# ChristophReich1996/Multi-StyleGAN

Measured on AMD Instinct MI355X. Metric: training images/sec (G+D step, 256^2, seq=3x2ch), higher is better.
Workload: dtype bf16

## Files before the change

include/msg_hip.h:

```cpp
#ifndef MSG_HIP_H
#define MSG_HIP_H

#ifdef __cplusplus
extern "C" {
#endif

enum { MSG_OK = 0, MSG_EINVAL = -1, MSG_EUNSUPPORTED = -2, MSG_ELAUNCH = -3 };
enum { MSG_F32 = 0, MSG_BF16 = 1, MSG_F16 = 2, MSG_F64 = 3, MSG_F32_SPLIT = 4 };

#define MSG_ABI_VERSION 5
int msg_abi_version(void);
const char* msg_build_arch(void);
const char* msg_strerror(int code);

int msg_upfirdn2d(const void* x, const float* fir, void* y, int dtype,
                  int major, int in_h, int in_w, int minor, int kh, int kw,
                  int up_x, int up_y, int down_x, int down_y,
                  int pad_x0, int pad_x1, int pad_y0, int pad_y1, void* stream);

int msg_upfirdn2d_pitched(const void* x, const float* fir, void* y, int dtype,
                          int major, int in_h, int in_w, int minor, int in_pitch, int kh, int kw,
                          int up_x, int up_y, int down_x, int down_y,
                          int pad_x0, int pad_x1, int pad_y0, int pad_y1, void* stream);

// ... 119 lines not shown

long long msg_minibatch_stddev_workspace(int C, int H, int W, int groups, int dtype);
int msg_minibatch_stddev(const void* x, void* y, float* stat, float* workspace, int dtype,
                         int B, int C, int H, int W, int ldx, int ldy, int groups, float alpha, void* stream);
int msg_minibatch_stddev_backward(const void* x, const void* gy, const float* gstat, void* gx, int dtype,
                                  int B, int C, int H, int W, int ldx, int ldgy, int ldgx, int groups,
                                  float alpha, void* stream);

int msg_conv2d_fprop_act(const void* x, const void* w, void* y, int dtype,
                         int B, int IH, int IW, int Cx, int Ck, int OH, int OW, int N, int ldy,
                         int kh, int kw, int stride, int pad, long long w_batch_stride,
                         const float* act_bias, const float* noise, const float* noise_weight,
                         int noise_batch, float alpha, float scale, void* stream);
int msg_conv2d_fprop_act_mask(const void* x, const void* w, void* y, int dtype,
                              int B, int IH, int IW, int Cx, int Ck, int OH, int OW, int N, int ldy,
                              int kh, int kw, int stride, int pad, long long w_batch_stride,
                              const float* act_bias, const float* noise, const float* noise_weight,
                              int noise_batch, float alpha, float scale, unsigned char* mask, void* stream);

int msg_conv2d_fprop_residual(const void* x, const void* w, void* y, int dtype,
                              int B, int IH, int IW, int Cx, int Ck, int OH, int OW, int N, int ldy,
                              int kh, int kw, int stride, int pad, long long w_batch_stride,
                              const void* residual, int res_ld, float gain, void* stream);

long long msg_conv2d_fprop_act_backward_workspace(int dtype, int B, int IH, int IW, int Cx, int Ck, int OH, int OW,
                                                  int N, int kh, int kw, long long w_batch_stride, int has_noise);
int msg_conv2d_fprop_act_backward(const void* x, const void* w, void* y, int dtype,
                                  int B, int IH, int IW, int Cx, int Ck, int OH, int OW, int N, int ldy,
                                  int kh, int kw, int stride, int pad, long long w_batch_stride,
                                  const void* residual, int res_ld,
                                  const unsigned char* sign_mask, int mask_tile_m, int mask_tile_n,
                                  const void* sign_map, int sign_ld, float alpha, float scale,
                                  float* grad_bias, const float* noise, int noise_batch, float* grad_noise_weight,
                                  float* ws, long long ws_floats, void* stream);

int msg_act_pointwise_head(const void* x, const float* bias, const float* w, float* y, int dtype,
                           long long npix, int C, float wscale, float alpha, float scale, void* stream);
long long msg_act_pointwise_head_backward_workspace(long long npix, int C);
int msg_act_pointwise_head_backward(const void* x, const float* bias, const float* w, const float* gy, void* gx,
                                    float* grad_bias_and_w, int dtype, long long npix, int C, float wscale,
                                    float alpha, float scale, float* ws, long long ws_floats, void* stream);

int msg_linear_fprop(const float* x, const float* w, const float* bias, float* y, int M, int N, int K,
                     float gain, float bias_gain, void* stream);
int msg_linear_dgrad(const float* gy, const float* w, float* gx, int M, int N, int K, float gain, void* stream);
int msg_linear_wgrad(const float* gy, const float* x, float* gw, float* gb, int M, int N, int K,
// ... 66 lines not shown
```

multi_stylegan_amd/conv_ops.py:

```python
import math
import os
from typing import Optional, Tuple

import torch
from torch.autograd import Function

from . import _lib
from ._autograd import _derive


def _vec(dtype) -> int:
    return 8 if dtype == torch.bfloat16 else 4


def _round_up(n: int, m: int) -> int:
    return (n + m - 1) // m * m


def _padded_nhwc(b, c, h, w, dtype, device):
    cx = _round_up(c, _vec(dtype))
    buf = torch.empty((b, h, w, cx), dtype=dtype, device=device)
    if cx != c:
        buf[..., c:].zero_()
    return buf.permute(0, 3, 1, 2)[:, :c]
# ... 315 lines not shown
        return self

    def __exit__(self, *exc):
        global FP32_CONTRACTION
        FP32_CONTRACTION = self.prev
        return False

    @staticmethod
    def set(mode: str) -> None:
        fp32_contraction(mode).__enter__()


def _contraction_code(t: torch.Tensor, mode: Optional[str] = None) -> int:
    code = _lib.dtype_code(t)
    mode = FP32_CONTRACTION if mode is None else mode
    return _SPLIT_CODES[mode] if (code == _lib.MSG_F32 and mode != "exact") else code


_PLANS = {_lib.MSG_PLAN_REG: ("conv_fprop_reg", None), _lib.MSG_PLAN_DMA: ("conv_fprop_dma", None),
          _lib.MSG_PLAN_PP: ("conv_fprop_pp", None), _lib.MSG_PLAN_ROW3: ("conv_fprop_row3", 256),
          _lib.MSG_PLAN_ROW3N: ("conv_fprop_row3n", 128), _lib.MSG_PLAN_THIN: ("conv_fprop_thin", None)}
_PLAN_CACHE: dict = {}
_WGRAD_WS_CACHE: dict = {}


def _launch_fprop(x, wk, ck, bias, n, out_hw, kh, kw, stride, pad, in_up, pixel_shuffle, per_sample, c_real,
                  flops=None, act=None, residual=None, out=None, mode=None):
    dev = _lib.require_gpu(x, wk, bias)
    xv, cx = _nhwc_view(x)
    b, _, ih, iw = xv.shape
    oh, ow = out_hw
    if out is not None:
        y, ldy = _nhwc_view(out)
        if y is not out or pixel_shuffle or out.shape != (b, n, oh, ow) or out.dtype != x.dtype or n % _vec(x.dtype):
            raise _lib.MsgHipError(f"conv fprop: destination {tuple(out.shape)} / {out.stride()} for a {(b, n, oh, ow)} result")
    elif pixel_shuffle:
        y, ldy = _alloc_out(b, n // 4, 2 * oh, 2 * ow, x.dtype, dev)
    else:
        y, ldy = _alloc_out(b, n, oh, ow, x.dtype, dev)
    rows_needed = n * (1 if pixel_shuffle else kh * kw) * ck
    if per_sample:
        ws_ = wk.stride() if wk.ndim == 4 else None
        if ws_ is None or wk.shape[0] != b or ws_[0] < rows_needed or ws_[3] != 1 or \
                (wk.shape[2] > 1 and ws_[2] != wk.shape[3]) or (wk.shape[1] > 1 and ws_[1] != wk.shape[2] * wk.shape[3]):
            raise _lib.MsgHipError(f"conv fprop: per-sample weight image {tuple(wk.shape)} for batch {b}, {n} x {kh * kw} x {ck}")
    elif wk.numel() < rows_needed or not wk.is_contiguous():
        raise _lib.MsgHipError(f"conv fprop: weight image {tuple(wk.shape)} smaller than {n} x {kh * kw} x {ck}")
    wstride = wk.stride(0) if per_sample else 0
    if flops is None:
        flops = 2.0 * b * oh * ow * n * kh * kw * c_real / (in_up * in_up)
    key = "conv_fprop"
    if _lib.kernel_clock.enabled:
        plan = _lib.lib().msg_conv2d_fprop_plan(_lib.dtype_code(x), b, ih, iw, cx, ck, oh, ow, n, kh, kw, wstride)
        key = _PLANS[_lib.MSG_PLAN_REG if plan == _lib.MSG_PLAN_THIN and act is not None else plan][0]
        if x.dtype == torch.bfloat16 and bias is None and act is None and residual is None and \
                _lib.lib().msg_conv2d_fprop_upconv_eligible(b, ih, iw, cx, ck, oh, ow, n, kh, kw, stride, pad, in_up,
                                                           int(pixel_shuffle), wstride):
            key = "conv_fprop_upconv"
        if _CLOCK_SHAPES:
            key += f"|B{b} {ih}x{iw}->{oh}x{ow} {c_real}->{n} {kh}x{kw} s{stride} up{in_up}" \
                   f"{' ps' if pixel_shuffle else ''}{' per-sample' if per_sample else ''}|"
    with _lib.on_device(dev), _lib.kernel_clock.span((key, 'bf16' if x.dtype == torch.bfloat16 else 'f32'), flops):
        if residual is not None:
            assert bias is None and act is None and in_up == 1 and not pixel_shuffle
            rv, res_ld = _nhwc_view(residual[0])
            assert rv.shape == (b, n, oh, ow) and rv.dtype == x.dtype
            code = _lib.lib().msg_conv2d_fprop_residual(
                xv.data_ptr(), wk.data_ptr(), y.data_ptr(), _contraction_code(x, mode), b, ih, iw, cx, ck, oh, ow, n, ldy, kh, kw,
                stride, pad, wstride, rv.data_ptr(), res_ld, float(residual[1]), _lib.stream_of(dev))
        elif act is None:
            code = _lib.lib().msg_conv2d_fprop(
                xv.data_ptr(), wk.data_ptr(), _lib.ptr(bias), y.data_ptr(), _contraction_code(x, mode), b, ih, iw, cx, ck, oh,
                ow, n, ldy, kh, kw, stride, pad, in_up, int(pixel_shuffle), wstride, _lib.stream_of(dev))
        else:
            assert bias is None and in_up == 1 and not pixel_shuffle
            act_bias, noise, noise_w, alpha, scale = act[:5]
            _lib.require_gpu(x, act_bias, noise, noise_w)
            mask = None
            if len(act) > 5 and act[5] is not None and kh == 3 and stride == 1 and pad == 1:
                pkey = (x.dtype, b, ih, iw, cx, ck, oh, ow, n, kh, kw, wstride)
                mplan = _PLAN_CACHE.get(pkey)
                if mplan is None:
                    mplan = _PLAN_CACHE[pkey] = _lib.lib().msg_conv2d_fprop_plan(_lib.dtype_code(x), b, ih, iw, cx, ck, oh, ow,
                                                                                n, kh, kw, wstride)
                tile = _PLANS[mplan][1]
                if tile:
                    from .op_static.fused_act import sign_mask_for
                    mask = sign_mask_for(b, n, oh, ow, x.dtype, dev)
                    if mask is not None:
                        act[5].append((mask, tile, tile))
            code = _lib.lib().msg_conv2d_fprop_act_mask(
                xv.data_ptr(), wk.data_ptr(), y.data_ptr(), _contraction_code(x, mode), b, ih, iw, cx, ck, oh, ow, n, ldy, kh, kw,
                stride, pad, wstride, _lib.ptr(act_bias), _lib.ptr(noise), _lib.ptr(noise_w),
                1 if noise is None else noise.shape[0], float(alpha), float(scale), _lib.ptr(mask), _lib.stream_of(dev))
    _lib.check(code, "msg_conv2d_fprop")
    return y


def _grad_dest(param):
    if param is None or "_msg_grad_slot" not in getattr(param, "__dict__", ()):
        return None
    from .dist import grad_destination
    return grad_destination(param)


def wgrad_k_chunks(b, o, i, taps, oh, ow, per_sample, kp):
    tiles = ((o + 127) // 128) * ((i + 127) // 128) * taps * b
    if per_sample:
        return max(1, min((oh * ow) // (16 * kp), 1024 // tiles)) if tiles < 256 else 1
    k_chunks = max(1, min((oh * ow + 4 * kp - 1) // (4 * kp), (1024 + tiles - 1) // tiles))
    while b * k_chunks > 65535:
        k_chunks -= 1
    return k_chunks


def _launch_wgrad(gy, x, o, i, kh, kw, stride, pad, pixel_shuffle, per_sample, low_hw, raw=False, gain=1.0, out=None,
                  mode=None):
# ... 1293 lines not shown
```

multi_stylegan_amd/csrc/conv_dispatch.h:

```cpp
#pragma once
#include "msg_common.h"

struct ConvProblem {
    int dtype;
    int split;
    int B, IH, IW, Cx, Ck, OH, OW, N, ldy;
    int kh, kw, stride, pad, in_up, pixel_shuffle;
    long long w_batch_stride;

    bool per_sample() const { return w_batch_stride != 0; }
    int samples() const { return per_sample() ? B : 1; }
    long long mtot() const { return per_sample() ? (long long)OH * OW : (long long)B * OH * OW; }
    int esz() const { return dtype == MSG_BF16 ? 2 : 4; }
    long long x_bstride() const { return (long long)IH * IW * Cx; }
    long long y_bstride() const { return (pixel_shuffle ? 4ll : 1ll) * OH * OW * ldy; }
    long long x_bytes() const { return (long long)(per_sample() ? 1 : B) * IH * IW * Cx * esz(); }
    long long w_bytes() const { return (long long)N * kh * kw * Ck * esz(); }
    bool fits31() const { return x_bytes() < 0x7ffffff0ll && w_bytes() < 0x7ffffff0ll; }
};

enum ConvKernel {
    CONV_THIN_N, CONV_THIN_K,
    CONV_UPCONV,
    CONV_ROW3, CONV_ROW3N,
    CONV_PP,
    CONV_DMA, CONV_REG, CONV_REG_LEAN, CONV_REG_SPLIT
};

struct ConvPlan {
    ConvKernel kernel;
    int tile_m, tile_n;
    bool supported;
};

inline int conv_act_mode(const ActEpilogue* act) { return act ? act->enabled : 0; }

template <typename P>
inline void conv_fill_common(P& p, const ConvProblem& q, const ActEpilogue* act) {
    p.B = q.B; p.IH = q.IH; p.IW = q.IW; p.Cx = q.Cx; p.Ck = q.Ck; p.OH = q.OH; p.OW = q.OW; p.N = q.N; p.ldy = q.ldy;
    p.per_sample = q.per_sample();
    if (act) p.act = *act;
    p.x_bstride = q.x_bstride();
    p.w_bstride = q.w_batch_stride;
    p.y_bstride = q.y_bstride();
    p.Mtot = (int)q.mtot();
}
template <typename P>
inline void conv_fill_taps(P& p, const ConvProblem& q) {
    p.kh = q.kh; p.kw = q.kw; p.stride = q.stride; p.pad = q.pad; p.in_up = q.in_up; p.pixel_shuffle = q.pixel_shuffle;
}

ConvPlan conv_fprop_select(const ConvProblem& q, const ActEpilogue* act, bool has_bias);

bool conv_thin_eligible(const ConvProblem& q, const ActEpilogue* act, ConvPlan* plan);
void conv_thin_launch(const ConvProblem& q, const ConvPlan& plan, const void* x, const void* w, const float* bias, void* y,
                      const ActEpilogue* act, void* stream);
bool conv_upconv_eligible(const ConvProblem& q, const ActEpilogue* act, bool has_bias, ConvPlan* plan);
void conv_upconv_launch(const ConvProblem& q, const ConvPlan& plan, const void* x, const void* w, void* y, void* stream);
bool conv_row3_eligible(const ConvProblem& q, const ActEpilogue* act, bool has_bias, ConvPlan* plan);
void conv_row3_launch(const ConvProblem& q, const ConvPlan& plan, const void* x, const void* w, const float* bias, void* y,
                      const ActEpilogue* act, void* stream);
bool conv_pp_eligible(const ConvProblem& q, ConvPlan* plan);
void conv_pp_launch(const ConvProblem& q, const ConvPlan& plan, const void* x, const void* w, const float* bias, void* y,
                    const ActEpilogue* act, void* stream);

struct WgradProblem {
    int dtype, split;
    int B, IH, IW, Cx, I, OH, OW, ldgy, O, ldgw;
    int kh, kw, stride, pad, pixel_shuffle;
    int per_sample, k_chunks, oi_major;
    float gain;
    int esz() const { return dtype == MSG_BF16 ? 2 : 4; }
    long long gy_bytes() const { return (long long)(pixel_shuffle ? 4 : 1) * OH * OW * ldgy * esz(); }
    long long x_bytes() const { return (long long)IH * IW * Cx * esz(); }
    long long slab() const { return (long long)O * kh * kw * ldgw; }
// ... 36 lines not shown
```

multi_stylegan_amd/csrc/conv_fprop.hip:

```cpp
#include "conv_dispatch.h"
#include <stdlib.h>

typedef __bf16 bf16v8 __attribute__((ext_vector_type(8)));
typedef const __attribute__((address_space(1))) char* gptr_t;
typedef const __attribute__((address_space(1))) u32x4* gvec_t;
typedef __attribute__((address_space(3))) char* lds_t;

struct ConvParams {
    int B, IH, IW, Cx, Ck, OH, OW, N, ldy;
    int kh, kw, stride, pad, in_up, pixel_shuffle, per_sample;
    long long x_bstride, w_bstride, y_bstride;
    int Mtot, n_chunks, n_iters, m_tiles, n_tiles;
    ActEpilogue act;
};

constexpr int BM = 128, BN = 128, ROWB = 128;
constexpr int STAGE_BYTES = (BM + BN) * ROWB;
__device__ __attribute__((aligned(256))) unsigned int g_zero_page[16384];

__device__ __forceinline__ int swz(int row, int slot) { return row * ROWB + ((slot ^ ((row >> 1) & 7)) << 4); }

template <int SPLIT>
__device__ __forceinline__ void split_park(const u32x4& raw, char* dst) {
    uint2 pl[3];
#pragma unroll
    for (int h = 0; h < 2; ++h) {
        const float x0 = __uint_as_float(raw[2 * h]), x1 = __uint_as_float(raw[2 * h + 1]);
        const unsigned hp = (unsigned)f2bf(x0) | ((unsigned)f2bf(x1) << 16);
        const float r0 = x0 - __uint_as_float(hp << 16), r1 = x1 - __uint_as_float(hp & 0xffff0000u);
        const unsigned mp = (unsigned)f2bf(r0) | ((unsigned)f2bf(r1) << 16);
        (h ? pl[0].y : pl[0].x) = hp;
        (h ? pl[1].y : pl[1].x) = mp;
        if constexpr (SPLIT == 3) {
            const float q0 = r0 - __uint_as_float(mp << 16), q1 = r1 - __uint_as_float(mp & 0xffff0000u);
            (h ? pl[2].y : pl[2].x) = (unsigned)f2bf(q0) | ((unsigned)f2bf(q1) << 16);
        }
    }
#pragma unroll
    for (int p = 0; p < SPLIT; ++p) *reinterpret_cast<uint2*>(dst + p * 64) = pl[p];
}

template <typename T, bool DMA, int LEAN = 0, int SPLIT = 0>
__global__ __launch_bounds__(256, LEAN ? LEAN : 2) void conv_fprop_kernel(const T* __restrict__ x, const T* __restrict__ w,
                                                            T* __restrict__ y, const float* __restrict__ bias,
                                                            ConvParams p) {
    constexpr int VEC = 16 / sizeof(T);
    constexpr int BKE = ROWB / sizeof(T);
    static_assert(!LEAN || (!DMA && sizeof(T) == 2), "lean variant: bf16, register staging");
    static_assert(SPLIT == 0 || sizeof(T) == 4, "split-bf16 products are a mode of the fp32-storage kernel");
    static_assert(SPLIT == 0 || !DMA, "the split planes are written from the staging registers");
    constexpr int SROW = SPLIT ? SPLIT * 64 + 16 : ROWB;
    constexpr int STAGE = SPLIT ? (BM + BN) * SROW : STAGE_BYTES;
    constexpr bool ONE_STAGE = LEAN != 0 || SPLIT == 3;
    constexpr int SMEM_BYTES = ONE_STAGE ? (STAGE > 65536 || sizeof(T) == 2 ? STAGE : 65536) : 2 * STAGE;
    __shared__ __attribute__((aligned(16))) char smem[SMEM_BYTES];

    const int tid = threadIdx.x, lane = tid & 63, wid = tid >> 6;
    const int wm = wid >> 1, wn = wid & 1;
    const int lr = lane & 31, lh = lane >> 5;
    const unsigned L = xcd_remap(blockIdx.x, gridDim.x);
    const int n0 = (int)(L % p.n_tiles) * BN;
    const int m0 = (int)(L / p.n_tiles) * BM;
    const int bz = blockIdx.z;

    const int wid_u = __builtin_amdgcn_readfirstlane(wid);
    const int slot_phys = tid & 7;
    int row_of[4];
#pragma unroll
    for (int j = 0; j < 4; ++j) row_of[j] = DMA ? (wid * 32 + 8 * j + (lane >> 3)) : ((tid >> 3) + 32 * j);
    const int slot = DMA ? 0 : slot_phys;
    int a_ih0[4], a_iw0[4];
    long long a_boff[4];
    int a_slot[4];
// ... 40 lines not shown
#pragma unroll
        for (int j = 0; j < 4; ++j) {
            const int n = n0 + row_of[j];
            vb[j] = n < p.N ? (int)(((long long)n * taps * p.Ck + a_slot[j] * VEC) * (long long)sizeof(T)) : MSG_DMA_OOB;
        }
    }
    const bool ragged = (p.Cx % BKE) != 0;
    int ld_tap = -1, ld_chunk = p.n_chunks - 1;
    int kh_ = 0, kw_ = -1;
    int st_off[4];
#pragma unroll
    for (int j = 0; j < 4; ++j) st_off[j] = swz(row_of[j], a_slot[j]);

    f32x16 acc[2][2];
#pragma unroll
    for (int i = 0; i < 2; ++i)
#pragma unroll
        for (int j = 0; j < 2; ++j)
#pragma unroll
            for (int e = 0; e < 16; ++e) acc[i][j][e] = 0.f;

    u32x4 ra[4], rb[4];
    int dma_stage = 0;
    auto load_next = [&]() __attribute__((always_inline)) {
        if (++ld_chunk == p.n_chunks) {
            ld_chunk = 0;
            ++ld_tap;
            if (++kw_ == p.kw) { kw_ = 0; ++kh_; }
            if (p.in_up == 1) {
                const long long tap_off = ((long long)kh_ * p.IW + kw_) * p.Cx * (long long)sizeof(T);
#pragma unroll
                for (int j = 0; j < 4; ++j) {
                    const bool ok = a_ok[j] & ((unsigned)(a_ih0[j] + kh_) < (unsigned)p.IH) &
                                    ((unsigned)(a_iw0[j] + kw_) < (unsigned)p.IW);
                    pa[j] = (ok ? xbase : zbase) + (ok ? a_boff[j] + tap_off : zoff);
                    if constexpr (DMA) va[j] = ok ? (int)(a_boff[j] + tap_off) : MSG_DMA_OOB;
                }
            } else {
#pragma unroll
                for (int j = 0; j < 4; ++j) {
                    const int ih = a_ih0[j] + kh_, iw = a_iw0[j] + kw_;
                    bool ok = a_ok[j] & (ih >= 0) & (iw >= 0) & (ih % p.in_up == 0) & (iw % p.in_up == 0);
                    const int ihs = ih / p.in_up, iws = iw / p.in_up;
                    ok = ok & (ihs < p.IH) & (iws < p.IW);
                    const long long off = a_boff[j] + ((long long)(ihs - a_ih0[j]) * p.IW + (iws - a_iw0[j])) * p.Cx * (long long)sizeof(T);
                    pa[j] = (ok ? xbase : zbase) + (ok ? off : zoff);
                    if constexpr (DMA) va[j] = ok ? (int)off : MSG_DMA_OOB;
                }
            }
        }
#pragma unroll
        for (int j = 0; j < 4; ++j) {
            const bool c_bad = ragged && (ld_chunk * BKE + a_slot[j] * VEC + VEC > p.Cx);
            gptr_t a_addr = pa[j];
            if (c_bad) a_addr = zbase + zoff;
            if constexpr (DMA) {
                const unsigned la = lds0 + dma_stage * STAGE + (wid_u * 32 + 8 * j) * ROWB;
                msg_dma16(d_x, la, c_bad ? MSG_DMA_OOB : va[j], ld_chunk * ROWB);
                msg_dma16(d_w, la + BM * ROWB, vb[j], (ld_tap * p.n_chunks + ld_chunk) * ROWB);
            } else {
                ra[j] = *(gvec_t)a_addr;
                rb[j] = *(gvec_t)pb[j];
            }
            pa[j] += ROWB;
            pb[j] += ROWB;
        }
    };
    auto park = [&](int stage) __attribute__((always_inline)) {
        char* sa = smem + stage * STAGE;
        if constexpr (SPLIT != 0) {
            char* sb = sa + BM * SROW;
#pragma unroll
// ... 62 lines not shown
                            for (int pa = 0; pa <= order; ++pa)
                                acc[i][j] = __builtin_amdgcn_mfma_f32_32x32x16_bf16(bf[order - pa][j], af[pa][i], acc[i][j], 0, 0, 0);
                    }
            }
        } else {
#pragma unroll
            for (int q = 0; q < 4; ++q) {
                f32x4 fa[2], fb[2];
#pragma unroll
                for (int t = 0; t < 2; ++t) {
                    fa[t] = *reinterpret_cast<const f32x4*>(sa + swz(wm * 64 + t * 32 + lr, 4 * lh + q));
                    fb[t] = *reinterpret_cast<const f32x4*>(sb + swz(wn * 64 + t * 32 + lr, 4 * lh + q));
                }
#pragma unroll
                for (int e = 0; e < 4; ++e)
#pragma unroll
                    for (int i = 0; i < 2; ++i)
#pragma unroll
                        for (int j = 0; j < 2; ++j)
                            acc[i][j] = __builtin_amdgcn_mfma_f32_32x32x2f32(fb[j][e], fa[i][e], acc[i][j], 0, 0, 0);
            }
        }
    };
    if constexpr (ONE_STAGE) {
        load_next();
        for (int it = 0; it < p.n_iters; ++it) {
            if (it) __syncthreads();
            park(0);
            if (it + 1 < p.n_iters) load_next();
            __syncthreads();
            mma_step(smem);
        }
    } else {
        if constexpr (DMA) {
            dma_stage = 0;
            load_next();
        } else {
            load_next();
            park(0);
            if (p.n_iters > 1) load_next();
        }
        for (int it = 0; it < p.n_iters; ++it) {
            if constexpr (DMA) asm volatile("s_waitcnt vmcnt(0)" ::: "memory");
            __syncthreads();
            if constexpr (DMA) {
                if (it + 1 < p.n_iters) { dma_stage = (it + 1) & 1; load_next(); }
            } else {
                if (it + 1 < p.n_iters) park((it + 1) & 1);
                if (it + 2 < p.n_iters) load_next();
            }
            mma_step(smem + (it & 1) * STAGE);
        }
    }
    if constexpr (DMA) asm volatile("s_waitcnt vmcnt(0)" ::: "memory");
    __syncthreads();

    constexpr int PITCH = 64 * sizeof(T);
    constexpr int UNITB = 4 * sizeof(T);
    char* ep = smem + wid * (64 * PITCH);
#pragma unroll
    for (int j = 0; j < 2; ++j)
#pragma unroll
        for (int g = 0; g < 4; ++g) {
            const int unit = 8 * j + 2 * g + lh;
            float bv[4] = {0.f, 0.f, 0.f, 0.f};
            if (bias) {
                const int nb = n0 + wn * 64 + 4 * unit;
#pragma unroll
                for (int e = 0; e < 4; ++e) bv[e] = nb + e < p.N ? bias[nb + e] : 0.f;
            }
#pragma unroll
            for (int i = 0; i < 2; ++i) {
                const int row = i * 32 + lr;
                char* dstl = ep + row * PITCH + ((unit ^ (row & 15)) * UNITB);
                if constexpr (sizeof(T) == 2) {
// ... 67 lines not shown
#pragma unroll
        for (int pass = 0; pass < NPASS; ++pass)
            r[pass] = *reinterpret_cast<const u32x4*>(rbase + (long long)max(gp[pass], 0) * p.act.res_ld);
#pragma unroll
        for (int pass = 0; pass < NPASS; ++pass) v[pass] = residual_epilogue_apply<T>(v[pass], r[pass], p.act.res_gain);
    }
    T* ybase = y + (p.pixel_shuffle ? nn : n);
    if (n_ok && lim >= VEC) {
#pragma unroll
        for (int pass = 0; pass < NPASS; ++pass)
            if (gp[pass] >= 0) *reinterpret_cast<u32x4*>(ybase + (long long)gp[pass] * p.ldy) = v[pass];
    } else if (n_ok) {
#pragma unroll
        for (int pass = 0; pass < NPASS; ++pass) {
            if (gp[pass] < 0) continue;
            T tmp[VEC];
            *reinterpret_cast<u32x4*>(tmp) = v[pass];
            T* dst = ybase + (long long)gp[pass] * p.ldy;
            for (int e = 0; e < lim; ++e) dst[e] = tmp[e];
        }
    }
}

static ConvPlan conv_generic_select(const ConvProblem& q) {
    const int n_iters = q.kh * q.kw * (q.Ck / (ROWB / q.esz()));
    static const int variant = msg_tunable("MSG_CONV_VARIANT", 0);
    const bool dma = q.fits31() && (variant == 1 || (variant == 0 && n_iters >= 8));
    static const int lean_max = msg_tunable("MSG_CONV_LEAN", 4);
    ConvPlan plan{CONV_REG, BM, BN, true};
    if (q.split) plan.kernel = CONV_REG_SPLIT;
    else if (dma) plan.kernel = CONV_DMA;
    else if (q.dtype == MSG_BF16 && n_iters <= lean_max) plan.kernel = CONV_REG_LEAN;
    const long long mtot = q.mtot(), blocks = ((mtot + BM - 1) / BM) * ((q.N + BN - 1) / BN);
    plan.supported = mtot < (1ll << 31) && blocks < (1ll << 31) &&
                     (long long)(n_iters + 1) * ROWB + 128 <= 65536;
    return plan;
}

static void conv_generic_launch(const ConvProblem& q, const ConvPlan& plan, const void* x, const void* w, const float* bias, void* y,
                                const ActEpilogue* act, void* stream) {
    ConvParams p{};
    conv_fill_common(p, q, act);
    conv_fill_taps(p, q);
    p.n_chunks = q.Ck / (ROWB / q.esz());
    p.n_iters = q.kh * q.kw * p.n_chunks;
    p.m_tiles = (int)((q.mtot() + BM - 1) / BM);
    p.n_tiles = (q.N + BN - 1) / BN;
    dim3 grid((unsigned)((long long)p.m_tiles * p.n_tiles), 1, q.samples());
#define GENERIC(T, ...) hipLaunchKernelGGL((conv_fprop_kernel<T, __VA_ARGS__>), grid, dim3(256), 0, (hipStream_t)stream, \
                                           (const T*)x, (const T*)w, (T*)y, bias, p)
    const bool bf16 = q.dtype == MSG_BF16;
    if (bf16 && plan.kernel == CONV_REG_LEAN) GENERIC(bf16_t, false, 3);
    else if (bf16 && plan.kernel == CONV_DMA) GENERIC(bf16_t, true);
    else if (bf16) GENERIC(bf16_t, false);
    else if (plan.kernel == CONV_REG_SPLIT) GENERIC(float, false, 0, 3);
    else if (plan.kernel == CONV_DMA) GENERIC(float, true);
    else GENERIC(float, false);
#undef GENERIC
}

ConvPlan conv_fprop_select(const ConvProblem& q, const ActEpilogue* act, bool has_bias) {
    ConvPlan plan;
    if (conv_thin_eligible(q, act, &plan)) return plan;
    if (conv_upconv_eligible(q, act, has_bias, &plan)) return plan;
    if (conv_row3_eligible(q, act, has_bias, &plan)) return plan;
    if (conv_pp_eligible(q, &plan)) return plan;
    return conv_generic_select(q);
}

static ConvProblem conv_problem(int dtype, int B, int IH, int IW, int Cx, int Ck, int OH, int OW, int N, int ldy,
                                int kh, int kw, int stride, int pad, int in_up, int pixel_shuffle, long long w_batch_stride) {
    const int split = dtype == MSG_F32_SPLIT ? 3 : 0;
    return ConvProblem{split ? (int)MSG_F32 : dtype, split, B, IH, IW, Cx, Ck, OH, OW, N, ldy, kh, kw, stride, pad, in_up, pixel_shuffle,
                       w_batch_stride};
}
static ConvProblem conv_query_problem(int dtype, int B, int IH, int IW, int Cx, int Ck, int OH, int OW, int N, int kh, int kw,
                                      long long w_batch_stride) {
    return conv_problem(dtype, B, IH, IW, Cx, Ck, OH, OW, N, N <= 8 ? 8 : (N + 7) / 8 * 8, kh, kw, 1, kh / 2, 1, 0, w_batch_stride);
}

extern "C" int msg_conv2d_fprop_plan(int dtype, int B, int IH, int IW, int Cx, int Ck, int OH, int OW, int N,
                                     int kh, int kw, long long w_batch_stride) {
    switch (conv_fprop_select(conv_query_problem(dtype, B, IH, IW, Cx, Ck, OH, OW, N, kh, kw, w_batch_stride), nullptr, false).kernel) {
        case CONV_THIN_N: case CONV_THIN_K: return MSG_PLAN_THIN;
        case CONV_ROW3: return MSG_PLAN_ROW3;
        case CONV_ROW3N: return MSG_PLAN_ROW3N;
        case CONV_PP: return MSG_PLAN_PP;
        case CONV_UPCONV: return MSG_PLAN_PP;
        case CONV_DMA: return MSG_PLAN_DMA;
        default: return MSG_PLAN_REG;
    }
}

static int conv2d_fprop_impl(const void* x, const void* w, const float* bias, void* y, const ConvProblem& q,
                             const ActEpilogue& act, void* stream, const ConvPlan* selected = nullptr);

extern "C" int msg_conv2d_fprop(const void* x, const void* w, const float* bias, void* y, int dtype,
                                int B, int IH, int IW, int Cx, int Ck, int OH, int OW, int N, int ldy,
                                int kh, int kw, int stride, int pad, int in_up, int pixel_shuffle,
                                long long w_batch_stride, void* stream) {
    ActEpilogue act{};
    return conv2d_fprop_impl(x, w, bias, y, conv_problem(dtype, B, IH, IW, Cx, Ck, OH, OW, N, ldy, kh, kw, stride, pad, in_up,
                                                         pixel_shuffle, w_batch_stride), act, stream);
}

static bool is_row3(const ConvPlan& plan) { return plan.kernel == CONV_ROW3 || plan.kernel == CONV_ROW3N; }

extern "C" int msg_conv2d_fprop_act_mask(const void* x, const void* w, void* y, int dtype,
                                         int B, int IH, int IW, int Cx, int Ck, int OH, int OW, int N, int ldy,
                                         int kh, int kw, int stride, int pad, long long w_batch_stride,
                                         const float* act_bias, const float* noise, const float* noise_weight,
                                         int noise_batch, float alpha, float scale, unsigned char* mask, void* stream) {
    if (noise && (!noise_weight || (noise_batch != 1 && noise_batch != B))) return MSG_EINVAL;
    const ConvProblem q = conv_problem(dtype, B, IH, IW, Cx, Ck, OH, OW, N, ldy, kh, kw, stride, pad, 1, 0, w_batch_stride);
    ActEpilogue act{act_bias, noise, noise_weight, noise_batch, 1, alpha, scale, nullptr, 0, 0.f, mask};
    if (!mask) return conv2d_fprop_impl(x, w, nullptr, y, q, act, stream);
    const ConvPlan plan = conv_fprop_select(q, &act, false);
    return is_row3(plan) ? conv2d_fprop_impl(x, w, nullptr, y, q, act, stream, &plan) : (int)MSG_EUNSUPPORTED;
}

extern "C" int msg_conv2d_fprop_act(const void* x, const void* w, void* y, int dtype,
                                    int B, int IH, int IW, int Cx, int Ck, int OH, int OW, int N, int ldy,
                                    int kh, int kw, int stride, int pad, long long w_batch_stride,
                                    const float* act_bias, const float* noise, const float* noise_weight,
                                    int noise_batch, float alpha, float scale, void* stream) {
    return msg_conv2d_fprop_act_mask(x, w, y, dtype, B, IH, IW, Cx, Ck, OH, OW, N, ldy, kh, kw, stride, pad, w_batch_stride,
// ... 49 lines not shown
    act_backward_partials(q, plan, &rows, &entries);
    if (!rows) return MSG_EUNSUPPORTED;
    if (sign_mask && (mask_tile_m <= 0 || mask_tile_n <= 0 || mask_tile_n % 128 || N % mask_tile_n || (((uintptr_t)sign_mask) & 15u) ||
                      (mask_tile_m != 1 && mask_tile_m % 64) || ((long long)B * OH * OW) % mask_tile_m))
        return MSG_EINVAL;
    if (sign_map && (sign_ld < N || sign_ld % 8 || (((uintptr_t)sign_map) & 15u))) return MSG_EINVAL;
    if (residual && (res_ld < N || res_ld % 8 || (((uintptr_t)residual) & 15u))) return MSG_EINVAL;
    const bool has_noise = noise && grad_noise_weight;
    if (has_noise && noise_batch != 1 && noise_batch != B) return MSG_EINVAL;
    const long long need_b = grad_bias ? rows * N : 0, need_n = has_noise ? entries : 0;
    if (need_b + need_n > 0 && (!ws || ws_floats < need_b + need_n)) return MSG_EINVAL;
    act.residual = residual; act.res_ld = res_ld; act.res_gain = 1.f;
    act.mask = const_cast<unsigned char*>(sign_mask); act.mask_tile_m = mask_tile_m; act.mask_tile_n = mask_tile_n;
    act.sign_src = sign_map; act.sign_ld = sign_ld;
    act.noise = has_noise ? noise : nullptr; act.noise_batch = noise_batch;
    act.part_b = grad_bias ? ws : nullptr;
    act.part_n = has_noise ? ws + need_b : nullptr;
    conv_row3_launch(q, plan, x, w, nullptr, y, &act, stream);
    if (MSG_CHECK_LAUNCH() != MSG_OK) return MSG_ELAUNCH;
    return msg_bias_act_reduce_launch(act.part_b, grad_bias, N, rows, act.part_n, grad_noise_weight, entries, stream);
}

static int conv2d_fprop_impl(const void* x, const void* w, const float* bias, void* y, const ConvProblem& q,
                             const ActEpilogue& act, void* stream, const ConvPlan* selected) {
    if (q.B == 0) return MSG_OK;
    if (!x || !w || !y || q.B < 0 || q.IH <= 0 || q.IW <= 0 || q.OH <= 0 || q.OW <= 0 || q.N <= 0 || q.kh <= 0 || q.kw <= 0 ||
        q.stride <= 0 || q.in_up <= 0 || q.Cx <= 0 || q.Ck <= 0 || q.ldy <= 0)
        return MSG_EINVAL;
    if (q.dtype != MSG_F32 && q.dtype != MSG_BF16) return MSG_EUNSUPPORTED;
    const int vec = 16 / q.esz(), bke = ROWB / q.esz();
    if (q.Ck % bke || q.Cx % vec || (((uintptr_t)x | (uintptr_t)w | (uintptr_t)y) & 15u)) return MSG_EUNSUPPORTED;
    if (q.ldy % vec || (q.pixel_shuffle && (q.N % 4 || (q.N / 4) % vec))) return MSG_EUNSUPPORTED;
    if (q.in_up > 1 && q.stride != 1) return MSG_EUNSUPPORTED;
    const ConvPlan plan = selected ? *selected : conv_fprop_select(q, &act, bias != nullptr);
    if (!plan.supported) return MSG_EUNSUPPORTED;
    switch (plan.kernel) {
        case CONV_THIN_N: case CONV_THIN_K: conv_thin_launch(q, plan, x, w, bias, y, &act, stream); break;
        case CONV_UPCONV: conv_upconv_launch(q, plan, x, w, y, stream); break;
        case CONV_ROW3: case CONV_ROW3N: conv_row3_launch(q, plan, x, w, bias, y, &act, stream); break;
        case CONV_PP: conv_pp_launch(q, plan, x, w, bias, y, &act, stream); break;
        case CONV_DMA: case CONV_REG: case CONV_REG_LEAN: case CONV_REG_SPLIT:
            conv_generic_launch(q, plan, x, w, bias, y, &act, stream); break;
    }
    return MSG_CHECK_LAUNCH();
}
```

Baseline: 156.9.

## Add split-K slabs with fp32 workspace reduction to generic conv fprop

Adds a split-K mode to the generic bf16 conv forward kernel. When a problem launches few workgroups but has a long K loop, each slice of K writes fp32 partial tiles to a workspace, and a finish kernel then sums the partials and applies bias, activation, residual or pixel-shuffle. The Python side now asks for the workspace size and passes scratch memory through new _ws entry points. The aim is to fill the GPU on small-spatial, deep-channel layers, at the cost of extra workspace traffic and a second launch.

Measured after the change: 157.5, median of 6. No clear change (+0.4%).

```diff
diff --git a/include/msg_hip.h b/include/msg_hip.h
--- a/include/msg_hip.h
+++ b/include/msg_hip.h
@@ -165,6 +165,25 @@
                               int B, int IH, int IW, int Cx, int Ck, int OH, int OW, int N, int ldy,
                               int kh, int kw, int stride, int pad, long long w_batch_stride,
                               const void* residual, int res_ld, float gain, void* stream);
+
+long long msg_conv2d_fprop_workspace(int dtype, int B, int IH, int IW, int Cx, int Ck, int OH, int OW, int N, int ldy,
+                                     int kh, int kw, int stride, int pad, int in_up, int pixel_shuffle,
+                                     long long w_batch_stride, int act_mode, int has_bias, int k_chunks);
+int msg_conv2d_fprop_ws(const void* x, const void* w, const float* bias, void* y, int dtype,
+                        int B, int IH, int IW, int Cx, int Ck, int OH, int OW, int N, int ldy,
+                        int kh, int kw, int stride, int pad, int in_up, int pixel_shuffle,
+                        long long w_batch_stride, int k_chunks, float* ws, long long ws_floats, void* stream);
+int msg_conv2d_fprop_act_ws(const void* x, const void* w, void* y, int dtype,
+                            int B, int IH, int IW, int Cx, int Ck, int OH, int OW, int N, int ldy,
+                            int kh, int kw, int stride, int pad, long long w_batch_stride,
+                            const float* act_bias, const float* noise, const float* noise_weight,
+                            int noise_batch, float alpha, float scale,
+                            int k_chunks, float* ws, long long ws_floats, void* stream);
+int msg_conv2d_fprop_residual_ws(const void* x, const void* w, void* y, int dtype,
+                                 int B, int IH, int IW, int Cx, int Ck, int OH, int OW, int N, int ldy,
+                                 int kh, int kw, int stride, int pad, long long w_batch_stride,
+                                 const void* residual, int res_ld, float gain,
+                                 int k_chunks, float* ws, long long ws_floats, void* stream);
 
 long long msg_conv2d_fprop_act_backward_workspace(int dtype, int B, int IH, int IW, int Cx, int Ck, int OH, int OW,
                                                   int N, int kh, int kw, long long w_batch_stride, int has_noise);
diff --git a/multi_stylegan_amd/conv_ops.py b/multi_stylegan_amd/conv_ops.py
--- a/multi_stylegan_amd/conv_ops.py
+++ b/multi_stylegan_amd/conv_ops.py
@@ -361,6 +361,14 @@
           _lib.MSG_PLAN_ROW3N: ("conv_fprop_row3n", 128), _lib.MSG_PLAN_THIN: ("conv_fprop_thin", None)}
 _PLAN_CACHE: dict = {}
 _WGRAD_WS_CACHE: dict = {}
+_FPROP_WS_CACHE: dict = {}
+
+
+def _fprop_workspace(dev, *geom):
+    need = _FPROP_WS_CACHE.get(geom)
+    if need is None:
+        need = _FPROP_WS_CACHE[geom] = _lib.lib().msg_conv2d_fprop_workspace(*geom)
+    return (_lib.scratch_ptr(need, dev), need) if need else (None, 0)
 
 
 def _launch_fprop(x, wk, ck, bias, n, out_hw, kh, kw, stride, pad, in_up, pixel_shuffle, per_sample, c_real,
@@ -399,18 +407,21 @@
         if _CLOCK_SHAPES:
             key += f"|B{b} {ih}x{iw}->{oh}x{ow} {c_real}->{n} {kh}x{kw} s{stride} up{in_up}" \
                    f"{' ps' if pixel_shuffle else ''}{' per-sample' if per_sample else ''}|"
+    ws, need = _fprop_workspace(dev, _contraction_code(x, mode), b, ih, iw, cx, ck, oh, ow, n, ldy, kh, kw, stride, pad, in_up,
+                                int(pixel_shuffle), wstride, 2 if residual is not None else int(act is not None),
+                                int(bias is not None), 0)
     with _lib.on_device(dev), _lib.kernel_clock.span((key, 'bf16' if x.dtype == torch.bfloat16 else 'f32'), flops):
         if residual is not None:
             assert bias is None and act is None and in_up == 1 and not pixel_shuffle
             rv, res_ld = _nhwc_view(residual[0])
             assert rv.shape == (b, n, oh, ow) and rv.dtype == x.dtype
-            code = _lib.lib().msg_conv2d_fprop_residual(
+            code = _lib.lib().msg_conv2d_fprop_residual_ws(
                 xv.data_ptr(), wk.data_ptr(), y.data_ptr(), _contraction_code(x, mode), b, ih, iw, cx, ck, oh, ow, n, ldy, kh, kw,
-                stride, pad, wstride, rv.data_ptr(), res_ld, float(residual[1]), _lib.stream_of(dev))
+                stride, pad, wstride, rv.data_ptr(), res_ld, float(residual[1]), 0, ws, need, _lib.stream_of(dev))
         elif act is None:
-            code = _lib.lib().msg_conv2d_fprop(
+            code = _lib.lib().msg_conv2d_fprop_ws(
                 xv.data_ptr(), wk.data_ptr(), _lib.ptr(bias), y.data_ptr(), _contraction_code(x, mode), b, ih, iw, cx, ck, oh,
-                ow, n, ldy, kh, kw, stride, pad, in_up, int(pixel_shuffle), wstride, _lib.stream_of(dev))
+                ow, n, ldy, kh, kw, stride, pad, in_up, int(pixel_shuffle), wstride, 0, ws, need, _lib.stream_of(dev))
         else:
             assert bias is None and in_up == 1 and not pixel_shuffle
             act_bias, noise, noise_w, alpha, scale = act[:5]
@@ -428,10 +439,16 @@
                     mask = sign_mask_for(b, n, oh, ow, x.dtype, dev)
                     if mask is not None:
                         act[5].append((mask, tile, tile))
-            code = _lib.lib().msg_conv2d_fprop_act_mask(
-                xv.data_ptr(), wk.data_ptr(), y.data_ptr(), _contraction_code(x, mode), b, ih, iw, cx, ck, oh, ow, n, ldy, kh, kw,
-                stride, pad, wstride, _lib.ptr(act_bias), _lib.ptr(noise), _lib.ptr(noise_w),
-                1 if noise is None else noise.shape[0], float(alpha), float(scale), _lib.ptr(mask), _lib.stream_of(dev))
+            if mask is None:
+                code = _lib.lib().msg_conv2d_fprop_act_ws(
+                    xv.data_ptr(), wk.data_ptr(), y.data_ptr(), _contraction_code(x, mode), b, ih, iw, cx, ck, oh, ow, n, ldy, kh,
+                    kw, stride, pad, wstride, _lib.ptr(act_bias), _lib.ptr(noise), _lib.ptr(noise_w),
+                    1 if noise is None else noise.shape[0], float(alpha), float(scale), 0, ws, need, _lib.stream_of(dev))
+            else:
+                code = _lib.lib().msg_conv2d_fprop_act_mask(
+                    xv.data_ptr(), wk.data_ptr(), y.data_ptr(), _contraction_code(x, mode), b, ih, iw, cx, ck, oh, ow, n, ldy, kh,
+                    kw, stride, pad, wstride, _lib.ptr(act_bias), _lib.ptr(noise), _lib.ptr(noise_w),
+                    1 if noise is None else noise.shape[0], float(alpha), float(scale), _lib.ptr(mask), _lib.stream_of(dev))
     _lib.check(code, "msg_conv2d_fprop")
     return y
 
diff --git a/multi_stylegan_amd/csrc/conv_dispatch.h b/multi_stylegan_amd/csrc/conv_dispatch.h
--- a/multi_stylegan_amd/csrc/conv_dispatch.h
+++ b/multi_stylegan_amd/csrc/conv_dispatch.h
@@ -31,6 +31,8 @@
     ConvKernel kernel;
     int tile_m, tile_n;
     bool supported;
+    int k_chunks = 1, k_steps = 0;
+    long long ws_floats = 0;
 };
 
 inline int conv_act_mode(const ActEpilogue* act) { return act ? act->enabled : 0; }
@@ -50,7 +52,7 @@
     p.kh = q.kh; p.kw = q.kw; p.stride = q.stride; p.pad = q.pad; p.in_up = q.in_up; p.pixel_shuffle = q.pixel_shuffle;
 }
 
-ConvPlan conv_fprop_select(const ConvProblem& q, const ActEpilogue* act, bool has_bias);
+ConvPlan conv_fprop_select(const ConvProblem& q, const ActEpilogue* act, bool has_bias, int k_req = 1);
 
 bool conv_thin_eligible(const ConvProblem& q, const ActEpilogue* act, ConvPlan* plan);
 void conv_thin_launch(const ConvProblem& q, const ConvPlan& plan, const void* x, const void* w, const float* bias, void* y,
diff --git a/multi_stylegan_amd/csrc/conv_fprop.hip b/multi_stylegan_amd/csrc/conv_fprop.hip
--- a/multi_stylegan_amd/csrc/conv_fprop.hip
+++ b/multi_stylegan_amd/csrc/conv_fprop.hip
@@ -12,6 +12,8 @@
     long long x_bstride, w_bstride, y_bstride;
     int Mtot, n_chunks, n_iters, m_tiles, n_tiles;
     ActEpilogue act;
+    int k_chunks, k_steps;
+    float* ws;
 };
 
 constexpr int BM = 128, BN = 128, ROWB = 128;
@@ -40,7 +42,7 @@
     for (int p = 0; p < SPLIT; ++p) *reinterpret_cast<uint2*>(dst + p * 64) = pl[p];
 }
 
-template <typename T, bool DMA, int LEAN = 0, int SPLIT = 0>
+template <typename T, bool DMA, int LEAN = 0, int SPLIT = 0, int SLAB = 0>
 __global__ __launch_bounds__(256, LEAN ? LEAN : 2) void conv_fprop_kernel(const T* __restrict__ x, const T* __restrict__ w,
                                                             T* __restrict__ y, const float* __restrict__ bias,
                                                             ConvParams p) {
@@ -49,6 +51,7 @@
     static_assert(!LEAN || (!DMA && sizeof(T) == 2), "lean variant: bf16, register staging");
     static_assert(SPLIT == 0 || sizeof(T) == 4, "split-bf16 products are a mode of the fp32-storage kernel");
     static_assert(SPLIT == 0 || !DMA, "the split planes are written from the staging registers");
+    static_assert(SLAB == 0 || (sizeof(T) == 2 && LEAN == 0 && SPLIT == 0), "K-chunk slabs: the plain bf16 instantiations");
     constexpr int SROW = SPLIT ? SPLIT * 64 + 16 : ROWB;
     constexpr int STAGE = SPLIT ? (BM + BN) * SROW : STAGE_BYTES;
     constexpr bool ONE_STAGE = LEAN != 0 || SPLIT == 3;
@@ -135,11 +138,7 @@
 
     u32x4 ra[4], rb[4];
     int dma_stage = 0;
-    auto load_next = [&]() __attribute__((always_inline)) {
-        if (++ld_chunk == p.n_chunks) {
-            ld_chunk = 0;
-            ++ld_tap;
-            if (++kw_ == p.kw) { kw_ = 0; ++kh_; }
+    auto set_tap = [&]() __attribute__((always_inline)) {
             if (p.in_up == 1) {
                 const long long tap_off = ((long long)kh_ * p.IW + kw_) * p.Cx * (long long)sizeof(T);
 #pragma unroll
@@ -161,6 +160,13 @@
                     if constexpr (DMA) va[j] = ok ? (int)off : MSG_DMA_OOB;
                 }
             }
+    };
+    auto load_next = [&]() __attribute__((always_inline)) {
+        if (++ld_chunk == p.n_chunks) {
+            ld_chunk = 0;
+            ++ld_tap;
+            if (++kw_ == p.kw) { kw_ = 0; ++kh_; }
+            set_tap();
         }
 #pragma unroll
         for (int j = 0; j < 4; ++j) {
@@ -269,12 +275,28 @@
             }
         }
     };
+    int n_it = p.n_iters;
+    if constexpr (SLAB) {
+        const int k0 = (int)blockIdx.y * p.k_steps;
+        n_it = min(p.k_steps, p.n_iters - k0);
+        ld_tap = k0 / p.n_chunks;
+        const int c0 = k0 - ld_tap * p.n_chunks;
+        kh_ = ld_tap / p.kw;
+        kw_ = ld_tap - kh_ * p.kw;
+        set_tap();
+#pragma unroll
+        for (int j = 0; j < 4; ++j) {
+            pa[j] += c0 * ROWB;
+            pb[j] += (long long)k0 * ROWB;
+        }
+        ld_chunk = c0 - 1;
+    }
     if constexpr (ONE_STAGE) {
         load_next();
-        for (int it = 0; it < p.n_iters; ++it) {
+        for (int it = 0; it < n_it; ++it) {
             if (it) __syncthreads();
             park(0);
-            if (it + 1 < p.n_iters) load_next();
+            if (it + 1 < n_it) load_next();
             __syncthreads();
             mma_step(smem);
         }
@@ -285,19 +307,37 @@
         } else {
             load_next();
             park(0);
-            if (p.n_iters > 1) load_next();
-        }
-        for (int it = 0; it < p.n_iters; ++it) {
+            if (n_it > 1) load_next();
+        }
+        for (int it = 0; it < n_it; ++it) {
             if constexpr (DMA) asm volatile("s_waitcnt vmcnt(0)" ::: "memory");
             __syncthreads();
             if constexpr (DMA) {
-                if (it + 1 < p.n_iters) { dma_stage = (it + 1) & 1; load_next(); }
+                if (it + 1 < n_it) { dma_stage = (it + 1) & 1; load_next(); }
             } else {
-                if (it + 1 < p.n_iters) park((it + 1) & 1);
-                if (it + 2 < p.n_iters) load_next();
+                if (it + 1 < n_it) park((it + 1) & 1);
+                if (it + 2 < n_it) load_next();
             }
             mma_step(smem + (it & 1) * STAGE);
         }
+    }
+    if constexpr (SLAB) {
+        if constexpr (DMA) asm volatile("s_waitcnt vmcnt(0)" ::: "memory");
+        const int npad = p.n_tiles * BN;
+        float* slab = p.ws + ((long long)blockIdx.y * gridDim.z + bz) * p.Mtot * npad;
+#pragma unroll
+        for (int i = 0; i < 2; ++i) {
+            const int row = m0 + wm * 64 + i * 32 + lr;
+            if (row >= p.Mtot) continue;
+            float* dst = slab + (long long)row * npad + n0 + wn * 64 + 4 * lh;
+#pragma unroll
+            for (int j = 0; j < 2; ++j)
+#pragma unroll
+                for (int g = 0; g < 4; ++g)
+                    *reinterpret_cast<f32x4*>(dst + 32 * j + 8 * g) =
+                        f32x4{acc[i][j][4 * g + 0], acc[i][j][4 * g + 1], acc[i][j][4 * g + 2], acc[i][j][4 * g + 3]};
+        }
+        return;
     }
     if constexpr (DMA) asm volatile("s_waitcnt vmcnt(0)" ::: "memory");
     __syncthreads();
@@ -411,7 +451,84 @@
     }
 }
 
-static ConvPlan conv_generic_select(const ConvProblem& q) {
+__global__ __launch_bounds__(256) void conv_ksplit_finish_kernel(bf16_t* __restrict__ y, const float* __restrict__ bias, ConvParams p) {
+    constexpr int VEC = 8;
+    const int npad = p.n_tiles * BN, vpr = npad / VEC;
+    const long long t = (long long)blockIdx.x * 256 + threadIdx.x;
+    if (t >= (long long)p.Mtot * vpr) return;
+    const int m = (int)(t / vpr), n = (int)(t - (long long)m * vpr) * VEC;
+    if (n >= p.N) return;
+    const int bz = blockIdx.z;
+    const long long cstride = (long long)gridDim.z * p.Mtot * npad;
+    const float* src = p.ws + ((long long)bz * p.Mtot + m) * npad + n;
+    f32x4 s0 = *reinterpret_cast<const f32x4*>(src), s1 = *reinterpret_cast<const f32x4*>(src + 4);
+#pragma unroll 4
+    for (int c = 1; c < p.k_chunks; ++c) {
+        src += cstride;
+        s0 += *reinterpret_cast<const f32x4*>(src);
+        s1 += *reinterpret_cast<const f32x4*>(src + 4);
+    }
+    float bv[VEC];
+#pragma unroll
+    for (int e = 0; e < VEC; ++e) bv[e] = (bias && n + e < p.N) ? bias[n + e] : 0.f;
+    u32x4 v;
+#pragma unroll
+    for (int h = 0; h < 2; ++h) {
+        const f32x4 a = h ? s1 : s0;
+        v[2 * h] = (unsigned)f2bf(a[0] + bv[4 * h + 0]) | ((unsigned)f2bf(a[1] + bv[4 * h + 1]) << 16);
+        v[2 * h + 1] = (unsigned)f2bf(a[2] + bv[4 * h + 2]) | ((unsigned)f2bf(a[3] + bv[4 * h + 3]) << 16);
+    }
+    const int ohw = p.OH * p.OW;
+    const int b = p.per_sample ? bz : m / ohw;
+    const int pix = p.per_sample ? m : m - b * ohw;
+    const int oh = pix / p.OW, ow = pix - oh * p.OW;
+    int nn = n, q = 0;
+    if (p.pixel_shuffle) { const int oc = p.N >> 2; q = n / oc; nn = n - q * oc; }
+    const int lim = p.pixel_shuffle ? (p.N >> 2) - nn : p.N - n;
+    const long long g = p.pixel_shuffle ? ((long long)(b * 2 * p.OH + 2 * oh + (q >> 1)) * (2 * p.OW) + 2 * ow + (q & 1))
+                                        : (long long)b * ohw + pix;
+    if (p.act.enabled == 1) {
+        float a_bias[VEC];
+#pragma unroll
+        for (int e = 0; e < VEC; ++e) a_bias[e] = (p.act.bias && n + e < p.N) ? p.act.bias[n + e] : 0.f;
+        const float a_noise = p.act.noise ? p.act.noise_w[0] * p.act.noise[(long long)(p.act.noise_batch == 1 ? 0 : b) * ohw + pix] : 0.f;
+        v = act_epilogue_apply<bf16_t>(v, a_bias, a_noise, p.act.alpha, p.act.scale);
+    } else if (p.act.enabled == 2) {
+        const u32x4 r = *reinterpret_cast<const u32x4*>(reinterpret_cast<const bf16_t*>(p.act.residual) + g * p.act.res_ld + n);
+        v = residual_epilogue_apply<bf16_t>(v, r, p.act.res_gain);
+    }
+    bf16_t* dst = y + g * p.ldy + nn;
+    if (lim >= VEC) {
+        *reinterpret_cast<u32x4*>(dst) = v;
+    } else {
+        bf16_t tmp[VEC];
+        *reinterpret_cast<u32x4*>(tmp) = v;
+        for (int e = 0; e < lim; ++e) dst[e] = tmp[e];
+    }
+}
+
+constexpr int KSPLIT_ROUND_WGS = 512;
+constexpr int KSPLIT_MIN_SWEEP = 32, KSPLIT_MIN_STEPS = 6, KSPLIT_MAX_CHUNKS = 64;
+constexpr long long KSPLIT_MAX_FLOATS = 16ll << 20;
+static int conv_generic_ksplit(long long wgs, int n_iters, long long slab_floats, int k_req) {
+    static const int enabled = msg_tunable("MSG_CONV_KSPLIT", 1);
+    static const int fixed_steps = msg_tunable("MSG_CONV_KSPLIT_FIXED", 8);
+    static const int slab_steps = msg_tunable("MSG_CONV_KSPLIT_SLAB", 4);
+    if (k_req == 1 || n_iters < 2) return 1;
+    if (k_req > 1) return k_req < n_iters ? (k_req < 65535 ? k_req : 65535) : n_iters;
+    if (!enabled || wgs > KSPLIT_ROUND_WGS / 2 || n_iters < KSPLIT_MIN_SWEEP) return 1;
+    int chunks = 1;
+    long long best = -1;
+    for (int c = 1; c <= KSPLIT_MAX_CHUNKS; ++c) {
+        if (c > 1 && (n_iters / c < KSPLIT_MIN_STEPS || c * slab_floats > KSPLIT_MAX_FLOATS)) break;
+        const long long rounds = (wgs * c + KSPLIT_ROUND_WGS - 1) / KSPLIT_ROUND_WGS;
+        const long long cost = rounds * ((n_iters + c - 1) / c + fixed_steps) + (c > 1 ? slab_steps * (1 + ((c * slab_floats) >> 20)) : 0);
+        if (best < 0 || cost < best) { best = cost; chunks = c; }
+    }
+    return chunks;
+}
+
+static ConvPlan conv_generic_select(const ConvProblem& q, int k_req) {
     const int n_iters = q.kh * q.kw * (q.Ck / (ROWB / q.esz()));
     static const int variant = msg_tunable("MSG_CONV_VARIANT", 0);
     const bool dma = q.fits31() && (variant == 1 || (variant == 0 && n_iters >= 8));
@@ -423,11 +540,21 @@
     const long long mtot = q.mtot(), blocks = ((mtot + BM - 1) / BM) * ((q.N + BN - 1) / BN);
     plan.supported = mtot < (1ll << 31) && blocks < (1ll << 31) &&
                      (long long)(n_iters + 1) * ROWB + 128 <= 65536;
+    if (plan.supported && q.dtype == MSG_BF16 && !q.split) {
+        const long long slab_floats = q.samples() * mtot * ((q.N + BN - 1) / BN * BN);
+        const int want = conv_generic_ksplit(blocks * q.samples(), n_iters, slab_floats, k_req);
+        if (want > 1 && (long long)want * slab_floats < (1ll << 40)) {
+            plan.k_steps = (n_iters + want - 1) / want;
+            plan.k_chunks = (n_iters + plan.k_steps - 1) / plan.k_steps;
+            plan.ws_floats = plan.k_chunks * slab_floats;
+            if (plan.kernel == CONV_REG_LEAN) plan.kernel = CONV_REG;
+        }
+    }
     return plan;
 }
 
 static void conv_generic_launch(const ConvProblem& q, const ConvPlan& plan, const void* x, const void* w, const float* bias, void* y,
-                                const ActEpilogue* act, void* stream) {
+                                const ActEpilogue* act, float* ws, void* stream) {
     ConvParams p{};
     conv_fill_common(p, q, act);
     conv_fill_taps(p, q);
@@ -435,11 +562,21 @@
     p.n_iters = q.kh * q.kw * p.n_chunks;
     p.m_tiles = (int)((q.mtot() + BM - 1) / BM);
     p.n_tiles = (q.N + BN - 1) / BN;
-    dim3 grid((unsigned)((long long)p.m_tiles * p.n_tiles), 1, q.samples());
+    p.k_chunks = plan.k_chunks;
+    p.k_steps = plan.k_steps;
+    p.ws = ws;
+    dim3 grid((unsigned)((long long)p.m_tiles * p.n_tiles), plan.k_chunks, q.samples());
 #define GENERIC(T, ...) hipLaunchKernelGGL((conv_fprop_kernel<T, __VA_ARGS__>), grid, dim3(256), 0, (hipStream_t)stream, \
                                            (const T*)x, (const T*)w, (T*)y, bias, p)
     const bool bf16 = q.dtype == MSG_BF16;
-    if (bf16 && plan.kernel == CONV_REG_LEAN) GENERIC(bf16_t, false, 3);
+    if (plan.k_chunks > 1) {
+        if (plan.kernel == CONV_DMA) GENERIC(bf16_t, true, 0, 0, 1);
+        else GENERIC(bf16_t, false, 0, 0, 1);
+        if (MSG_CHECK_LAUNCH() != MSG_OK) return;
+        const long long vecs = (long long)p.Mtot * (p.n_tiles * BN / 8);
+        hipLaunchKernelGGL(conv_ksplit_finish_kernel, dim3((unsigned)((vecs + 255) / 256), 1, q.samples()), dim3(256), 0,
+                           (hipStream_t)stream, (bf16_t*)y, bias, p);
+    } else if (bf16 && plan.kernel == CONV_REG_LEAN) GENERIC(bf16_t, false, 3);
     else if (bf16 && plan.kernel == CONV_DMA) GENERIC(bf16_t, true);
     else if (bf16) GENERIC(bf16_t, false);
     else if (plan.kernel == CONV_REG_SPLIT) GENERIC(float, false, 0, 3);
@@ -448,13 +585,13 @@
 #undef GENERIC
 }
 
-ConvPlan conv_fprop_select(const ConvProblem& q, const ActEpilogue* act, bool has_bias) {
+ConvPlan conv_fprop_select(const ConvProblem& q, const ActEpilogue* act, bool has_bias, int k_req) {
     ConvPlan plan;
     if (conv_thin_eligible(q, act, &plan)) return plan;
     if (conv_upconv_eligible(q, act, has_bias, &plan)) return plan;
     if (conv_row3_eligible(q, act, has_bias, &plan)) return plan;
     if (conv_pp_eligible(q, &plan)) return plan;
-    return conv_generic_select(q);
+    return conv_generic_select(q, k_req);
 }
 
 static ConvProblem conv_problem(int dtype, int B, int IH, int IW, int Cx, int Ck, int OH, int OW, int N, int ldy,
@@ -482,7 +619,8 @@
 }
 
 static int conv2d_fprop_impl(const void* x, const void* w, const float* bias, void* y, const ConvProblem& q,
-                             const ActEpilogue& act, void* stream, const ConvPlan* selected = nullptr);
+                             const ActEpilogue& act, void* stream, const ConvPlan* selected = nullptr, int k_req = 1,
+                             float* ws = nullptr, long long ws_floats = 0);
 
 extern "C" int msg_conv2d_fprop(const void* x, const void* w, const float* bias, void* y, int dtype,
                                 int B, int IH, int IW, int Cx, int Ck, int OH, int OW, int N, int ldy,
@@ -491,6 +629,53 @@
     ActEpilogue act{};
     return conv2d_fprop_impl(x, w, bias, y, conv_problem(dtype, B, IH, IW, Cx, Ck, OH, OW, N, ldy, kh, kw, stride, pad, in_up,
                                                          pixel_shuffle, w_batch_stride), act, stream);
+}
+
+extern "C" long long msg_conv2d_fprop_workspace(int dtype, int B, int IH, int IW, int Cx, int Ck, int OH, int OW, int N, int ldy,
+                                                int kh, int kw, int stride, int pad, int in_up, int pixel_shuffle,
+                                                long long w_batch_stride, int act_mode, int has_bias, int k_chunks) {
+    if (B <= 0 || IH <= 0 || IW <= 0 || OH <= 0 || OW <= 0 || N <= 0 || kh <= 0 || kw <= 0 || stride <= 0 || in_up <= 0 || Cx <= 0 ||
+        Ck <= 0 || ldy <= 0 || k_chunks < 0 || (dtype != MSG_BF16 && dtype != MSG_F32 && dtype != MSG_F32_SPLIT))
+        return 0;
+    const ConvProblem q = conv_problem(dtype, B, IH, IW, Cx, Ck, OH, OW, N, ldy, kh, kw, stride, pad, in_up, pixel_shuffle, w_batch_stride);
+    if (q.Ck % (ROWB / q.esz())) return 0;
+    ActEpilogue act{};
+    act.enabled = act_mode;
+    return conv_fprop_select(q, &act, has_bias != 0, k_chunks).ws_floats;
+}
+
+extern "C" int msg_conv2d_fprop_ws(const void* x, const void* w, const float* bias, void* y, int dtype,
+                                   int B, int IH, int IW, int Cx, int Ck, int OH, int OW, int N, int ldy,
+                                   int kh, int kw, int stride, int pad, int in_up, int pixel_shuffle,
+                                   long long w_batch_stride, int k_chunks, float* ws, long long ws_floats, void* stream) {
+    if (k_chunks < 0) return MSG_EINVAL;
+    ActEpilogue act{};
+    return conv2d_fprop_impl(x, w, bias, y, conv_problem(dtype, B, IH, IW, Cx, Ck, OH, OW, N, ldy, kh, kw, stride, pad, in_up,
+                                                         pixel_shuffle, w_batch_stride), act, stream, nullptr, k_chunks, ws, ws_floats);
+}
+
+extern "C" int msg_conv2d_fprop_act_ws(const void* x, const void* w, void* y, int dtype,
+                                       int B, int IH, int IW, int Cx, int Ck, int OH, int OW, int N, int ldy,
+                                       int kh, int kw, int stride, int pad, long long w_batch_stride,
+                                       const float* act_bias, const float* noise, const float* noise_weight,
+                                       int noise_batch, float alpha, float scale,
+                                       int k_chunks, float* ws, long long ws_floats, void* stream) {
+    if (k_chunks < 0 || (noise && (!noise_weight || (noise_batch != 1 && noise_batch != B)))) return MSG_EINVAL;
+    ActEpilogue act{act_bias, noise, noise_weight, noise_batch, 1, alpha, scale, nullptr, 0, 0.f, nullptr};
+    return conv2d_fprop_impl(x, w, nullptr, y, conv_problem(dtype, B, IH, IW, Cx, Ck, OH, OW, N, ldy, kh, kw, stride, pad, 1, 0,
+                                                            w_batch_stride), act, stream, nullptr, k_chunks, ws, ws_floats);
+}
+
+extern "C" int msg_conv2d_fprop_residual_ws(const void* x, const void* w, void* y, int dtype,
+                                            int B, int IH, int IW, int Cx, int Ck, int OH, int OW, int N, int ldy,
+                                            int kh, int kw, int stride, int pad, long long w_batch_stride,
+                                            const void* residual, int res_ld, float gain,
+                                            int k_chunks, float* ws, long long ws_floats, void* stream) {
+    if (k_chunks < 0 || !residual || res_ld < N || (((uintptr_t)residual) & 15u) || res_ld % (dtype == MSG_BF16 ? 8 : 4)) return MSG_EINVAL;
+    ActEpilogue act{};
+    act.enabled = 2; act.residual = residual; act.res_ld = res_ld; act.res_gain = gain;
+    return conv2d_fprop_impl(x, w, nullptr, y, conv_problem(dtype, B, IH, IW, Cx, Ck, OH, OW, N, ldy, kh, kw, stride, pad, 1, 0,
+                                                            w_batch_stride), act, stream, nullptr, k_chunks, ws, ws_floats);
 }
 
 static bool is_row3(const ConvPlan& plan) { return plan.kernel == CONV_ROW3 || plan.kernel == CONV_ROW3N; }
@@ -586,7 +771,7 @@
 }
 
 static int conv2d_fprop_impl(const void* x, const void* w, const float* bias, void* y, const ConvProblem& q,
-                             const ActEpilogue& act, void* stream, const ConvPlan* selected) {
+                             const ActEpilogue& act, void* stream, const ConvPlan* selected, int k_req, float* ws, long long ws_floats) {
     if (q.B == 0) return MSG_OK;
     if (!x || !w || !y || q.B < 0 || q.IH <= 0 || q.IW <= 0 || q.OH <= 0 || q.OW <= 0 || q.N <= 0 || q.kh <= 0 || q.kw <= 0 ||
         q.stride <= 0 || q.in_up <= 0 || q.Cx <= 0 || q.Ck <= 0 || q.ldy <= 0)
@@ -596,15 +781,16 @@
     if (q.Ck % bke || q.Cx % vec || (((uintptr_t)x | (uintptr_t)w | (uintptr_t)y) & 15u)) return MSG_EUNSUPPORTED;
     if (q.ldy % vec || (q.pixel_shuffle && (q.N % 4 || (q.N / 4) % vec))) return MSG_EUNSUPPORTED;
     if (q.in_up > 1 && q.stride != 1) return MSG_EUNSUPPORTED;
-    const ConvPlan plan = selected ? *selected : conv_fprop_select(q, &act, bias != nullptr);
+    const ConvPlan plan = selected ? *selected : conv_fprop_select(q, &act, bias != nullptr, k_req);
     if (!plan.supported) return MSG_EUNSUPPORTED;
+    if (plan.k_chunks > 1 && (!ws || ws_floats < plan.ws_floats || (((uintptr_t)ws) & 15u))) return MSG_EINVAL;
     switch (plan.kernel) {
         case CONV_THIN_N: case CONV_THIN_K: conv_thin_launch(q, plan, x, w, bias, y, &act, stream); break;
         case CONV_UPCONV: conv_upconv_launch(q, plan, x, w, y, stream); break;
         case CONV_ROW3: case CONV_ROW3N: conv_row3_launch(q, plan, x, w, bias, y, &act, stream); break;
         case CONV_PP: conv_pp_launch(q, plan, x, w, bias, y, &act, stream); break;
         case CONV_DMA: case CONV_REG: case CONV_REG_LEAN: case CONV_REG_SPLIT:
-            conv_generic_launch(q, plan, x, w, bias, y, &act, stream); break;
+            conv_generic_launch(q, plan, x, w, bias, y, &act, ws, stream); break;
     }
     return MSG_CHECK_LAUNCH();
 }
```
